# lvxianwei/DeepMerge

Hardware: NVIDIA B200
Metric: megapixels/sec end-to-end (RAG+pool+score+merge+relabel) (higher is better)
Workload: dtype int32/u8 index + fp32 scores

## Files before the change

### deepmerge_b200/csrc/rag_blocks.cu

```cuda
#include "rag_tables.cuh"

namespace dm {
namespace rag {
namespace blk {

template <int C_, int TH_, int NS_, int NW_, int ICAP_>
struct Cfg {
    static constexpr int C = C_, TH = TH_, NS = NS_, NWARPS = NW_, ICAP = ICAP_;
    static constexpr int CW = C_ > 0 ? C_ : 1;
    static constexpr int THREADS = NWARPS * 32;
    static constexpr int LAB_BOX = align128(TH * LAB_PITCH * 4);
    static constexpr int IMG_ROW_WORDS = STRIP_W * C / 4;
    static constexpr int IMG_BOX = align128(TH * IMG_ROW_WORDS * 4);
    static constexpr int STAGE_BYTES = LAB_BOX + IMG_BOX;
    static constexpr int ITEM_VECS = 7 + C;
    static constexpr int ITEM_BYTES = ICAP * ITEM_VECS * 16;
    static constexpr int TABLE_WORDS = RS * (3 + 2 * C) + ES * 3 + 4;
    static constexpr int TABLE_BYTES = align128(TABLE_WORDS * 4 + NS * 8);
    static constexpr int WARP_BYTES = NS * STAGE_BYTES + ITEM_BYTES + TABLE_BYTES;
    static constexpr int SMEM_BYTES = 128 + NWARPS * WARP_BYTES;
    static constexpr int TX_BYTES = TH * LAB_PITCH * 4 + (C > 0 ? TH * IMG_ROW_WORDS * 4 : 0);
    static constexpr int FLUSH_UNITS = FLUSH_ROWS / TH > 0 ? FLUSH_ROWS / TH : 1;
    static_assert(TH % 4 == 0, "a stage holds whole block rows");
    static_assert(ICAP % 8 == 0 && ICAP >= 40, "item buffer: the rest of a pass (< 32 items) plus a block row of new ones");
    static_assert(SMEM_BYTES <= 227 * 1024, "shared memory budget");
};

__device__ __noinline__ void slow_wait(uint64_t* bar, unsigned parity, unsigned long long* counters) {
    mbar_wait(bar, parity, counters);
}

template <typename CF>
__device__ __noinline__ void item_pass(uint4* items, unsigned* tab, const Params* Pp, int icount, int lane) {
    constexpr int C = CF::C, CW = CF::CW, ICAP = CF::ICAP;
    const Params& P = *Pp;
    const Tab<C> T = Tab<C>::from(tab);
    __syncwarp();
    const int n = min(32, icount), base = icount - n;
    if (lane < n) {
        const int j = base + lane;
        const uint4* it = items + j;
        int lab[ragcore::WIN];
        unsigned img[4 * CW];
        uint4 v = it[0];
        lab[20] = (int)v.x; lab[21] = (int)v.y; lab[22] = (int)v.z; lab[23] = (int)v.w;
#pragma unroll
        for (int r = 0; r < 4; ++r) {
            v = it[(1 + r) * ICAP];
            lab[5 * r] = (int)v.x; lab[5 * r + 1] = (int)v.y; lab[5 * r + 2] = (int)v.z; lab[5 * r + 3] = (int)v.w;
        }
        v = it[5 * ICAP];
        lab[4] = (int)v.x; lab[9] = (int)v.y; lab[14] = (int)v.z; lab[19] = (int)v.w;
#pragma unroll
        for (int vi = 0; vi < C; ++vi) {
            v = it[(6 + vi) * ICAP];
            img[4 * vi] = v.x; img[4 * vi + 1] = v.y; img[4 * vi + 2] = v.z; img[4 * vi + 3] = v.w;
        }
        v = it[(6 + C) * ICAP];
        const ragcore::Geo g{P.W, P.rows_own, P.rows_avail, P.top_border, P.bottom_border};
        Sink<C> sink{T, P};
        const ItemPick<ICAP> pick{(const int*)items, j};
        ragcore::process_item<C>(lab, img, (int)v.x, (int)v.y, g, sink, pick);
    }
    __syncwarp();
}

template <typename CF, bool USE_TMA>
__global__ void __launch_bounds__(CF::THREADS, 1)
rag_blocks_kernel(const __grid_constant__ CUtensorMap mapL, const __grid_constant__ CUtensorMap mapI,
                  const __grid_constant__ Params P) {
    constexpr int C = CF::C, CW = CF::CW, TH = CF::TH, NS = CF::NS, ICAP = CF::ICAP;
    extern __shared__ __align__(128) unsigned char smem_raw[];
    unsigned char* smem = smem_raw + ((128u - (smem_u32(smem_raw) & 127u)) & 127u);
    const int warp = __shfl_sync(0xffffffffu, (int)(threadIdx.x >> 5), 0);
    const int lane = threadIdx.x & 31;
    unsigned char* wbase = smem + (size_t)warp * CF::WARP_BYTES;
    uint4* items = (uint4*)(wbase + NS * CF::STAGE_BYTES);
    unsigned* tab = (unsigned*)(wbase + NS * CF::STAGE_BYTES + CF::ITEM_BYTES);
    const Tab<C> T = Tab<C>::from(tab);
    uint64_t* full_bar = (uint64_t*)(tab + ((CF::TABLE_WORDS + 1) & ~1));

    const long long total_units = (long long)P.tiles_x * P.tiles_y;
    const long long gw = (long long)blockIdx.x * CF::NWARPS + warp;
    const long long n_warps = (long long)gridDim.x * CF::NWARPS;
    const long long u_begin = total_units / n_warps * gw + min(gw, total_units % n_warps);
    const long long u_end = u_begin + total_units / n_warps + (gw < total_units % n_warps ? 1 : 0);
    const int my_units = (int)(u_end - u_begin);

    T.rkey[lane] = EMPTY_LABEL;
    T.rarea[lane] = 0;
    T.rborder[lane] = 0;
#pragma unroll
    for (int c = 0; c < C; ++c) {
        T.rsum[c * RS + lane] = 0;
        T.rsq[c * RS + lane] = 0;
    }
    T.ekey[lane] = EMPTY_KEY;
    T.ekey[lane + 32] = EMPTY_KEY;
    T.ecnt[lane] = 0;
    T.ecnt[lane + 32] = 0;
    if (lane == 0) {
        T.used[0] = T.used[1] = 0;
        if (USE_TMA) {
            for (int s = 0; s < NS; ++s) mbar_init(&full_bar[s], 1);
            asm volatile("fence.mbarrier_init.release.cluster;" ::: "memory");
        }
    }
    __syncwarp();
    if (my_units == 0) return;

    int isx = (int)(u_begin / P.tiles_y), ij = (int)(u_begin - (long long)isx * P.tiles_y), issued = 0;
    auto issue = [&]() {
        if (lane == 0) {
            const int st = issued % NS;
            unsigned char* sb = wbase + (size_t)st * CF::STAGE_BYTES;
            mbar_expect_tx(&full_bar[st], (unsigned)CF::TX_BYTES);
            tma_load_2d(sb, &mapL, isx * STRIP_W, ij * TH, &full_bar[st]);
            if (C > 0) tma_load_2d(sb + CF::LAB_BOX, &mapI, isx * STRIP_W * C / 4, ij * TH, &full_bar[st]);
        }
        ++issued;
        if (ij + 1 < P.tiles_y) ++ij;
        else { ij = 0; ++isx; }
    };
    if (USE_TMA) {
        for (int k = 0; k < NS && k < my_units; ++k) issue();
    }

    int4 up = make_int4(0, 0, 0, 0);
    int cur = EMPTY_LABEL;
    unsigned area = 0, s[CW], q[CW];
#pragma unroll
    for (int c = 0; c < CW; ++c) s[c] = q[c] = 0;
    int icount = 0;
    auto lane_flush = [&]() {
        if (cur >= 0 && area) table_region_add<C>(T, P, cur, area, 0u, s, q);
        area = 0;
#pragma unroll
        for (int c = 0; c < CW; ++c) s[c] = q[c] = 0;
    };

    int units_since_flush = 0;
    int sx = (int)(u_begin / P.tiles_y), j = (int)(u_begin - (long long)sx * P.tiles_y);
    bool contiguous = false;

    for (int i = 0; i < my_units; ++i) {
        const int st = USE_TMA ? i % NS : 0;
        unsigned char* sb = wbase + (size_t)st * CF::STAGE_BYTES;
        const int strip_x0 = sx * STRIP_W, unit_y0 = j * TH;
        int* Lw = (int*)sb;
        if (USE_TMA) {
            if (!mbar_try_wait(&full_bar[st], (unsigned)(i / NS) & 1u)) slow_wait(&full_bar[st], (unsigned)(i / NS) & 1u, P.counters);
        } else {
            __syncwarp();
            for (int k = lane; k < TH * LAB_PITCH; k += 32) {
                const int r = k / LAB_PITCH, cidx = k - r * LAB_PITCH;
                const int gy = unit_y0 + r, gx = strip_x0 + cidx;
                Lw[k] = (gy < P.rows_avail && gx < P.W) ? P.labels[(int64_t)gy * P.ld + gx] : 0;
            }
            if constexpr (C > 0) {
                unsigned char* Ib = sb + CF::LAB_BOX;
                for (int k = lane; k < TH * CF::IMG_ROW_WORDS * 4; k += 32) {
                    const int r = k / (CF::IMG_ROW_WORDS * 4), bidx = k - r * (CF::IMG_ROW_WORDS * 4);
                    const int gy = unit_y0 + r;
                    const int64_t gb = (int64_t)strip_x0 * C + bidx;
                    Ib[k] = (gy < P.rows_own && gb < (int64_t)P.W * C) ? P.image[(int64_t)gy * P.image_pitch + gb] : 0;
                }
            }
            __syncwarp();
        }

        const int x0 = strip_x0 + 4 * lane;
        const bool in_img = x0 < P.W;
        const bool forced_x = (x0 == 0) || (x0 + 4 >= P.W);
        if (!contiguous) {
            up = make_int4(0, 0, 0, 0);
            if (unit_y0 > 0) {
                const int32_t* row = P.labels + (int64_t)(unit_y0 - 1) * P.ld;
                if (x0 < P.W) up.x = row[x0];
                if (x0 + 1 < P.W) up.y = row[x0 + 1];
                if (x0 + 2 < P.W) up.z = row[x0 + 2];
                if (x0 + 3 < P.W) up.w = row[x0 + 3];
            }
        }

#pragma unroll
        for (int b = 0; b < TH / 4; ++b) {
            const int y0 = unit_y0 + 4 * b;
            if (y0 >= P.rows_avail) break;
            const int* Lp = Lw + (4 * b) * LAB_PITCH + 4 * lane;
            const int4 a0 = *(const int4*)Lp;
            const int4 a1 = *(const int4*)(Lp + LAB_PITCH);
            const int4 a2 = *(const int4*)(Lp + 2 * LAB_PITCH);
            const int4 a3 = *(const int4*)(Lp + 3 * LAB_PITCH);
            int r0 = __shfl_down_sync(0xffffffffu, a0.x, 1);
            int r1 = __shfl_down_sync(0xffffffffu, a1.x, 1);
            int r2 = __shfl_down_sync(0xffffffffu, a2.x, 1);
            int r3 = __shfl_down_sync(0xffffffffu, a3.x, 1);
            if (lane == 31) {
                r0 = Lp[4];
                r1 = Lp[LAB_PITCH + 4];
                r2 = Lp[2 * LAB_PITCH + 4];
                r3 = Lp[3 * LAB_PITCH + 4];
            }
            unsigned px[4][CW];
            if constexpr (C > 0) {
                const unsigned* Ip = (const unsigned*)(sb + CF::LAB_BOX) + (4 * b) * CF::IMG_ROW_WORDS + CW * lane;
#pragma unroll
                for (int r = 0; r < 4; ++r) {
                    if constexpr (C == 4) {
                        const uint4 v = *(const uint4*)(Ip + r * CF::IMG_ROW_WORDS);
                        px[r][0] = v.x; px[r][1] = v.y; px[r][2] = v.z; px[r][3] = v.w;
                    } else {
#pragma unroll
                        for (int c = 0; c < C; ++c) px[r][c] = Ip[r * CF::IMG_ROW_WORDS + c];
                    }
                }
            }
            const unsigned d = or3(or3(or3(eq3(up.x, up.y, up.z), eq3(up.z, up.w, a0.x), eq3(a0.x, a0.y, a0.z)),
                                       or3(eq3(a0.z, a0.w, r0), eq3(r0, a1.x, a1.y), eq3(a1.y, a1.z, a1.w)),
                                       or3(eq3(a1.w, r1, a2.x), eq3(a2.x, a2.y, a2.z), eq3(a2.z, a2.w, r2))),
                                   or3(eq3(r2, a3.x, a3.y), eq3(a3.y, a3.z, a3.w), eq3(a3.w, r3, up.x)), 0u);
            const bool forced = forced_x || (y0 == 0) || (y0 + 4 >= P.rows_own);
            const bool is_item = in_img && (forced || d != 0u);
            const bool is_fast = in_img && !is_item;
            const int ref = a0.x;
            if (is_fast && ref != cur) {
                lane_flush();
                cur = ref;
            }
            __syncwarp();
            if (is_fast) {
                area += 16u;
                if constexpr (C > 0) {
#pragma unroll
                    for (int r = 0; r < 4; ++r) ragcore::row_stats<C>(px[r], s, q);
                }
            }
            const unsigned bal = __ballot_sync(0xffffffffu, is_item);
            if (bal) {
                if (icount + __popc(bal) > ICAP) {
                    item_pass<CF>(items, tab, &P, icount, lane);
                    icount -= min(32, icount);
                }
                if (is_item) {
                    uint4* it = items + (icount + __popc(bal & lanemask_lt()));
                    it[0] = make_uint4((unsigned)up.x, (unsigned)up.y, (unsigned)up.z, (unsigned)up.w);
                    it[1 * ICAP] = make_uint4((unsigned)a0.x, (unsigned)a0.y, (unsigned)a0.z, (unsigned)a0.w);
                    it[2 * ICAP] = make_uint4((unsigned)a1.x, (unsigned)a1.y, (unsigned)a1.z, (unsigned)a1.w);
                    it[3 * ICAP] = make_uint4((unsigned)a2.x, (unsigned)a2.y, (unsigned)a2.z, (unsigned)a2.w);
                    it[4 * ICAP] = make_uint4((unsigned)a3.x, (unsigned)a3.y, (unsigned)a3.z, (unsigned)a3.w);
                    it[5 * ICAP] = make_uint4((unsigned)r0, (unsigned)r1, (unsigned)r2, (unsigned)r3);
                    if constexpr (C > 0) {
                        const unsigned* Wf = &px[0][0];
#pragma unroll
                        for (int vi = 0; vi < C; ++vi)
                            it[(6 + vi) * ICAP] = make_uint4(Wf[4 * vi], Wf[4 * vi + 1], Wf[4 * vi + 2], Wf[4 * vi + 3]);
                    }
                    it[(6 + C) * ICAP] = make_uint4((unsigned)x0, (unsigned)y0, 0u, 0u);
                }
                icount += __popc(bal);
            }
            up = a3;
        }
        contiguous = (j + 1 < P.tiles_y);

        if (j + 1 < P.tiles_y) ++j;
        else { j = 0; ++sx; }

        __syncwarp();
        if (USE_TMA && i + NS < my_units) {
            asm volatile("fence.proxy.async.shared::cta;" ::: "memory");
            issue();
        }

        ++units_since_flush;
        const bool forced_flush = units_since_flush >= CF::FLUSH_UNITS || (i + 1 == my_units);
        if (icount >= 32 || forced_flush) {
            while (icount >= 32 || (forced_flush && icount > 0)) {
                item_pass<CF>(items, tab, &P, icount, lane);
                icount -= min(32, icount);
                if (icount > 0 && (T.used[0] > RS / 2 || T.used[1] > ES / 2)) drain_tables<C>(tab, &P, lane);
            }
            if (forced_flush) {
                lane_flush();
                units_since_flush = 0;
            }
        }
        __syncwarp();
        const uint2 used = *(const uint2*)T.used;
        if (forced_flush || used.x > RS / 2 || used.y > ES / 2) drain_tables<C>(tab, &P, lane);
    }
}

template <typename CF>
static int run(const Params& Pin, cudaStream_t s) {
    Params P = Pin;
    P.tiles_x = (int)ceil_div(P.W, STRIP_W);
    P.tiles_y = (int)ceil_div(P.rows_avail, CF::TH);
    const long long total = (long long)P.tiles_x * P.tiles_y;
    if (total == 0) return DM_OK;
    const long long max_warps = (long long)num_sms() * CF::NWARPS;
    const long long per = ceil_div(total, max_warps);
    if (per > 0x7fffffff) return DM_ERR_BAD_ARG;
    P.tiles_per_cta = (int)per;
    const int grid = (int)imin64(num_sms(), ceil_div(total, CF::NWARPS));

    CUtensorMap mapL, mapI;
    memset(&mapL, 0, sizeof(mapL));
    memset(&mapI, 0, sizeof(mapI));
    bool tma = ((uintptr_t)P.labels % 16 == 0) && ((P.ld * 4) % 16 == 0) && P.ld >= P.W;
    if (CF::C > 0)
        tma = tma && ((uintptr_t)P.image % 16 == 0) && (P.image_pitch % 16 == 0) && (((int64_t)P.W * CF::C) % 4 == 0);
    if (tma)
        tma = make_map_2d(&mapL, P.labels, (uint64_t)P.W, (uint64_t)P.rows_avail, (uint64_t)P.ld * 4, LAB_PITCH, CF::TH);
    if (tma && CF::C > 0)
        tma = make_map_2d(&mapI, P.image, (uint64_t)P.W * CF::C / 4, (uint64_t)P.rows_own, (uint64_t)P.image_pitch,
                          CF::IMG_ROW_WORDS, CF::TH);
    set_last_path(tma ? 1 : 0);
    return launch(tma ? rag_blocks_kernel<CF, true> : rag_blocks_kernel<CF, false>, grid, CF::THREADS, CF::SMEM_BYTES, s,
                  mapL, mapI, P);
}

}

int run_blocks(const Params& P, int C, cudaStream_t s) {
    using namespace blk;
    switch (C) {
        case 0: return run<Cfg<0, 8, 2, 14, 48>>(P, s);
        case 1: return run<Cfg<1, 4, 2, 16, 48>>(P, s);
        case 2: return run<Cfg<2, 4, 2, 14, 48>>(P, s);
        case 3: return run<Cfg<3, 4, 2, 12, 48>>(P, s);
        case 4: return run<Cfg<4, 4, 2, 12, 48>>(P, s);
        default: return DM_ERR_BAD_ARG;
    }
}

}
}
```

### deepmerge_b200/csrc/rag_core.cuh

```cuda
#pragma once
#include <stdint.h>

#if defined(__CUDACC__)
#define DM_HD __host__ __device__ __forceinline__
#else
#define DM_HD inline
#endif

namespace dm {
namespace ragcore {

DM_HD unsigned popc32(unsigned x) {
#if defined(__CUDA_ARCH__)
    return (unsigned)__popc(x);
#else
    return (unsigned)__builtin_popcount(x);
#endif
}
DM_HD int ffs32(unsigned x) {
#if defined(__CUDA_ARCH__)
    return __ffs((int)x);
#else
    return x ? __builtin_ctz(x) + 1 : 0;
#endif
}
DM_HD unsigned dp4a_u8(unsigned a, unsigned b, unsigned c) {
#if defined(__CUDA_ARCH__)
    return __dp4a(a, b, c);
#else
    for (int i = 0; i < 4; ++i) c += ((a >> (8 * i)) & 0xffu) * ((b >> (8 * i)) & 0xffu);
    return c;
#endif
}
DM_HD unsigned byte_perm(unsigned a, unsigned b, unsigned s) {
#if defined(__CUDA_ARCH__)
    return __byte_perm(a, b, s);
#else
    const unsigned long long v = ((unsigned long long)b << 32) | a;
    unsigned r = 0;
    for (int i = 0; i < 4; ++i) r |= (unsigned)((v >> (8 * ((s >> (4 * i)) & 7))) & 0xffu) << (8 * i);
    return r;
#endif
}

constexpr int WIN = 24;
constexpr unsigned OWN_BITS = 0x7BDEFu;
constexpr unsigned COL0_BITS = 0x08421u;
constexpr unsigned RIGHT_BITS = 0x84210u;
DM_HD unsigned row_bits(int n) { return (1u << (5 * n)) - 1u; }

struct Geo {
    int W, rows_own, rows_avail, top_border, bottom_border;
};

struct BlockMasks {
    unsigned PV;
    unsigned SV;
    unsigned HV;
    unsigned VV;
    unsigned SIDES[4];
};

DM_HD int clamp04(int v) { return v < 0 ? 0 : (v > 4 ? 4 : v); }

DM_HD BlockMasks block_masks(int x0, int y0, const Geo& g) {
    BlockMasks m;
    const int ncols = clamp04(g.W - x0);
    const int nh = clamp04(g.W - x0 - 1);
    const int nown = clamp04(g.rows_own - y0);
    const int nav = clamp04(g.rows_avail - y0);
    const unsigned cols = ((1u << ncols) - 1u) * COL0_BITS;
    m.SV = cols & row_bits(nown);
    const unsigned ownv = cols & row_bits(nav);
    const unsigned rightv = (x0 + 4 < g.W) ? (RIGHT_BITS & row_bits(nown)) : 0u;
    const unsigned upv = (y0 > 0) ? (((1u << ncols) - 1u) << 20) : 0u;
    m.PV = ownv | rightv | upv;
    m.HV = (((1u << nh) - 1u) * COL0_BITS) & row_bits(nown);
    m.VV = ownv & ~(y0 > 0 ? 0u : 0x1Fu);
    const int klast = g.W - 1 - x0, rlast = g.rows_own - 1 - y0;
    m.SIDES[0] = x0 == 0 ? COL0_BITS : 0u;
    m.SIDES[1] = (klast >= 0 && klast < 4) ? (COL0_BITS << klast) : 0u;
    m.SIDES[2] = (y0 == 0 && g.top_border) ? 0xFu : 0u;
    m.SIDES[3] = (rlast >= 0 && rlast < 4 && g.rows_avail == g.rows_own && g.bottom_border) ? (0xFu << (5 * rlast)) : 0u;
    return m;
}

DM_HD bool block_forced(int x0, int y0, const Geo& g) {
    return x0 == 0 || x0 + 4 >= g.W || y0 == 0 || y0 + 4 >= g.rows_own;
}

DM_HD unsigned upper_of(unsigned M) { return (((M & OWN_BITS) << 5) & OWN_BITS) | ((M >> 20) & 0xFu); }

DM_HD unsigned pairs_between(unsigned A, unsigned B, const BlockMasks& m) {
    const unsigned h = ((A & (B >> 1)) | (B & (A >> 1))) & m.HV;
    const unsigned v = ((A & upper_of(B)) | (B & upper_of(A))) & m.VV;
    return popc32(h) + popc32(v);
}

DM_HD unsigned nibble_to_bytes(unsigned nib) { return ((nib * 0x00204081u) & 0x01010101u) * 0xFFu; }

template <int C>
DM_HD void band_transpose(const unsigned* W, unsigned* T) {
    if constexpr (C == 4) {
        const unsigned t0 = byte_perm(W[0], W[1], 0x5140), t1 = byte_perm(W[0], W[1], 0x7362);
        const unsigned t2 = byte_perm(W[2], W[3], 0x5140), t3 = byte_perm(W[2], W[3], 0x7362);
        T[0] = byte_perm(t0, t2, 0x5410);
        T[1] = byte_perm(t0, t2, 0x7632);
        T[2] = byte_perm(t1, t3, 0x5410);
        T[3] = byte_perm(t1, t3, 0x7632);
    } else {
#if defined(__CUDA_ARCH__)
#pragma unroll
#endif
        for (int c = 0; c < C; ++c) {
            const int i0 = c, i1 = C + c, i2 = 2 * C + c, i3 = 3 * C + c;
            const unsigned t01 = byte_perm(W[i0 >> 2], W[i1 >> 2], (unsigned)((i0 & 3) | ((4 + (i1 & 3)) << 4)));
            const unsigned t23 = byte_perm(W[i2 >> 2], W[i3 >> 2], (unsigned)((i2 & 3) | ((4 + (i3 & 3)) << 4)));
            T[c] = byte_perm(t01, t23, 0x5410);
        }
    }
}

template <int C>
DM_HD void row_stats(const unsigned* W, unsigned* s, unsigned* q) {
    unsigned T[C > 0 ? C : 1];
    band_transpose<C>(W, T);
#if defined(__CUDA_ARCH__)
#pragma unroll
#endif
    for (int c = 0; c < C; ++c) {
        s[c] = dp4a_u8(T[c], 0x01010101u, s[c]);
        q[c] = dp4a_u8(T[c], T[c], q[c]);
    }
}

DM_HD unsigned window_spread(const int* lab) {
    unsigned d = 0;
#if defined(__CUDA_ARCH__)
#pragma unroll
#endif
    for (int p = 1; p < WIN; p += 2) {
        const unsigned a = (unsigned)lab[p - 1], b = (unsigned)lab[p], c = (unsigned)lab[(p + 1) % WIN];
        d |= (a ^ b) | (b ^ c);
    }
    return d;
}

template <int C, class Sink, class Pick>
DM_HD void process_item(const int* lab, const unsigned* img , int x0, int y0, const Geo& g, Sink& sink,
                        const Pick& pick) {
    constexpr int CW = C > 0 ? C : 1;
    const BlockMasks m = block_masks(x0, y0, g);

    unsigned MN = 0;
    {
        int any = 0;
#if defined(__CUDA_ARCH__)
#pragma unroll
#endif
        for (int p = 0; p < WIN; ++p) any |= lab[p];
        if (any < 0) {
#if defined(__CUDA_ARCH__)
#pragma unroll
#endif
            for (int p = 0; p < WIN; ++p) MN |= (lab[p] < 0 ? 1u : 0u) << p;
            MN &= m.PV;
        }
    }

    unsigned T[4][CW];
    if (C > 0) {
#if defined(__CUDA_ARCH__)
#pragma unroll
#endif
        for (int r = 0; r < 4; ++r) band_transpose<C>(img + r * CW, T[r]);
    }

    constexpr int MAXL = 4;
    unsigned rem = m.PV & ~MN;
    int Lq1 = 0, Lq2 = 0, Lq3 = 0;
    unsigned Mq1 = 0, Mq2 = 0, Mq3 = 0;
#if defined(__CUDA_ARCH__)
#pragma unroll 1
#endif
    for (int i = 0; i < MAXL && rem != 0; ++i) {
        const int l = pick(ffs32(rem) - 1);
        unsigned mm = 0;
#if defined(__CUDA_ARCH__)
#pragma unroll
#endif
        for (int p = 0; p < WIN; ++p) mm |= (lab[p] == l ? 1u : 0u) << p;
        mm &= rem;
        rem &= ~mm;
        {
            const unsigned ms = mm & m.SV;
            unsigned sides = popc32(ms & m.SIDES[0]) + popc32(ms & m.SIDES[1]) + popc32(ms & m.SIDES[2]) +
                             popc32(ms & m.SIDES[3]);
            if (MN) sides += pairs_between(mm, MN, m);
            unsigned s[CW], q[CW];
#if defined(__CUDA_ARCH__)
#pragma unroll
#endif
            for (int c = 0; c < CW; ++c) s[c] = q[c] = 0;
            if (C > 0) {
#if defined(__CUDA_ARCH__)
#pragma unroll
#endif
                for (int r = 0; r < 4; ++r) {
                    const unsigned bm = nibble_to_bytes((ms >> (5 * r)) & 0xFu);
#if defined(__CUDA_ARCH__)
#pragma unroll
#endif
                    for (int c = 0; c < C; ++c) {
                        const unsigned w = T[r][c] & bm;
                        s[c] = dp4a_u8(w, 0x01010101u, s[c]);
                        q[c] = dp4a_u8(w, w, q[c]);
                    }
                }
            }
            const unsigned area = popc32(ms);
            if (area | sides) sink.region(l, area, sides, s, q);
        }
#if defined(__CUDA_ARCH__)
#pragma unroll 1
#endif
        for (int j = 0; j < 3; ++j) {
            if (Mq1) {
                const unsigned n = pairs_between(mm, Mq1, m);
                if (n) sink.edge(l, Lq1, n);
            }
            const int tl = Lq1;
            const unsigned tm = Mq1;
            Lq1 = Lq2; Mq1 = Mq2;
            Lq2 = Lq3; Mq2 = Mq3;
            Lq3 = tl; Mq3 = tm;
        }
        Lq3 = Lq2; Mq3 = Mq2;
        Lq2 = Lq1; Mq2 = Mq1;
        Lq1 = l; Mq1 = mm;
    }
    if (rem == 0) return;

#if defined(__CUDA_ARCH__)
#pragma unroll
#endif
    for (int r = 0; r < 4; ++r) {
#if defined(__CUDA_ARCH__)
#pragma unroll 1
#endif
        for (int k = 0; k < 4; ++k) {
            const int p = 5 * r + k;
            const unsigned bit = 1u << p;
            const int l = pick(p);
            if ((m.SV & rem & bit) && l >= 0) {
                unsigned s[CW], q[CW];
                for (int c = 0; c < CW; ++c) s[c] = q[c] = 0;
                if (C > 0) {
                    const unsigned bm = 0xFFu << (8 * k);
                    for (int c = 0; c < C; ++c) {
                        const unsigned w = T[r][c] & bm;
                        s[c] = dp4a_u8(w, 0x01010101u, 0u);
                        q[c] = dp4a_u8(w, w, 0u);
                    }
                }
                const unsigned sides = ((m.SIDES[0] & bit) ? 1u : 0u) + ((m.SIDES[1] & bit) ? 1u : 0u) +
                                       ((m.SIDES[2] & bit) ? 1u : 0u) + ((m.SIDES[3] & bit) ? 1u : 0u);
                sink.region_slow(l, 1u, sides, s, q);
            }
            for (int which = 0; which < 2; ++which) {
                const bool ok = which == 0 ? (m.HV & bit) != 0 : (m.VV & bit) != 0;
                if (!ok) continue;
                const int po = which == 0 ? p + 1 : (r == 0 ? 20 + k : p - 5);
                if (((bit | (1u << po)) & rem) == 0) continue;
                const int o = pick(po);
                if (o == l) continue;
                if ((o | l) >= 0) {
                    sink.edge_slow(l, o, 1u);
                } else {
                    const int v = l >= 0 ? l : o;
                    if (v >= 0) {
                        unsigned z[CW];
                        for (int c = 0; c < CW; ++c) z[c] = 0;
                        sink.region_slow(v, 0u, 1u, z, z);
                    }
                }
            }
        }
    }
}

}
}
```

### deepmerge_b200/csrc/rag_tables.cuh

```cuda
#pragma once
#include "rag_common.cuh"
#include "rag_core.cuh"

namespace dm {
namespace rag {
namespace blk {

template <int C>
struct Tab {
    int* rkey;
    unsigned* rarea;
    unsigned* rborder;
    unsigned* rsum;
    unsigned* rsq;
    unsigned long long* ekey;
    unsigned* ecnt;
    unsigned* used;
    unsigned* base;

    __device__ __forceinline__ static Tab from(unsigned* tab) {
        Tab T;
        T.base = tab;
        T.rkey = (int*)tab;
        T.rarea = tab + RS;
        T.rborder = tab + 2 * RS;
        T.rsum = tab + 3 * RS;
        T.rsq = tab + (3 + C) * RS;
        T.ekey = (unsigned long long*)(tab + (3 + 2 * C) * RS);
        T.ecnt = tab + (3 + 2 * C) * RS + 2 * ES;
        T.used = tab + (3 + 2 * C) * RS + 3 * ES;
        return T;
    }
};

__device__ __forceinline__ unsigned eq3(int a, int b, int c) {
    unsigned d;
    asm("lop3.b32 %0, %1, %2, %3, 0x7E;" : "=r"(d) : "r"(a), "r"(b), "r"(c));
    return d;
}
__device__ __forceinline__ unsigned or3(unsigned a, unsigned b, unsigned c) {
    unsigned d;
    asm("lop3.b32 %0, %1, %2, %3, 0xFE;" : "=r"(d) : "r"(a), "r"(b), "r"(c));
    return d;
}
__device__ __forceinline__ void red_add_u64(unsigned long long* p, unsigned long long v) {
    asm volatile("red.global.add.u64 [%0], %1;" ::"l"(p), "l"(v) : "memory");
}

__device__ __forceinline__ int region_slot(int* rkey, unsigned* used, int label) {
    unsigned h = ((unsigned)label * 0x9E3779B1u) >> (32 - 5);
    static_assert(RS == 32, "hash shift");
#pragma unroll 1
    for (int p = 0; p < RS; ++p) {
        int k = rkey[h];
        if (k == label) return (int)h;
        if (k == EMPTY_LABEL) {
            int old = atomicCAS(&rkey[h], EMPTY_LABEL, label);
            if (old == EMPTY_LABEL) {
                atomicAdd(&used[0], 1u);
                return (int)h;
            }
            if (old == label) return (int)h;
        }
        h = (h + 1) & (RS - 1);
    }
    return SLOT_NONE;
}

__device__ __forceinline__ void raw_append(const Params& P, unsigned long long key, unsigned cnt) {
    if ((long long)key_hi(key) >= P.n_regions) {
        atomicExch(&P.counters[3], 1ull);
        return;
    }
    unsigned long long i = atomicAdd(&P.counters[1], 1ull);
    if ((long long)i < P.capacity) {
        P.raw_keys[i] = key;
        P.raw_cnt[i] = cnt;
    } else {
        atomicExch(&P.counters[2], 1ull);
    }
}

template <int C>
__device__ __forceinline__ void edge_add(const Tab<C>& T, const Params& P, unsigned long long key, unsigned cnt) {
    unsigned h = (((unsigned)(key >> 32) * 0x9E3779B1u) ^ ((unsigned)key * 0x85EBCA6Bu)) >> (32 - 6);
    static_assert(ES == 64, "hash shift");
#pragma unroll 1
    for (int p = 0; p < ES / 2; ++p) {
        unsigned long long k = T.ekey[h];
        if (k == EMPTY_KEY) {
            k = atomicCAS(&T.ekey[h], EMPTY_KEY, key);
            if (k == EMPTY_KEY) {
                atomicAdd(&T.used[1], 1u);
                k = key;
            }
        }
        if (k == key) {
            atomicAdd(&T.ecnt[h], cnt);
            return;
        }
        h = (h + 1) & (ES - 1);
    }
    raw_append(P, key, cnt);
}

template <int C>
__device__ __forceinline__ void global_region_add(const Params& P, int label, unsigned area, unsigned border,
                                                  const unsigned* s, const unsigned* q) {
    if ((unsigned)label >= (unsigned)P.n_regions) {
        atomicExch(&P.counters[3], 1ull);
        return;
    }
    if (area) red_add_u64(&P.area[label], (unsigned long long)area);
    if (border) red_add_u64(&P.border[label], (unsigned long long)border);
    if (C > 0 && area) {
#pragma unroll
        for (int c = 0; c < C; ++c) {
            red_add_u64(&P.bsum[(size_t)label * C + c], (unsigned long long)s[c]);
            red_add_u64(&P.bsq[(size_t)label * C + c], (unsigned long long)q[c]);
        }
    }
}

template <int C>
__device__ __noinline__ void global_region_add_slow(const Params* P, int label, unsigned area, unsigned border, uint4 s4,
                                                    uint4 q4) {
    const unsigned s[4] = {s4.x, s4.y, s4.z, s4.w}, q[4] = {q4.x, q4.y, q4.z, q4.w};
    global_region_add<C>(*P, label, area, border, s, q);
}

template <int C>
__device__ __forceinline__ void table_region_add(const Tab<C>& T, const Params& P, int label, unsigned area,
                                                 unsigned border, const unsigned* s, const unsigned* q) {
    const int slot = region_slot(T.rkey, T.used, label);
    if (slot >= 0) {
        if (area) atomicAdd(&T.rarea[slot], area);
        if (border) atomicAdd(&T.rborder[slot], border);
        if (C > 0 && area) {
#pragma unroll
            for (int c = 0; c < C; ++c) {
                atomicAdd(&T.rsum[c * RS + slot], s[c]);
                atomicAdd(&T.rsq[c * RS + slot], q[c]);
            }
        }
    } else {
        uint4 s4 = make_uint4(0, 0, 0, 0), q4 = make_uint4(0, 0, 0, 0);
        if (C > 0) { s4.x = s[0]; q4.x = q[0]; }
        if (C > 1) { s4.y = s[1 % (C > 0 ? C : 1)]; q4.y = q[1 % (C > 0 ? C : 1)]; }
        if (C > 2) { s4.z = s[2 % (C > 0 ? C : 1)]; q4.z = q[2 % (C > 0 ? C : 1)]; }
        if (C > 3) { s4.w = s[3 % (C > 0 ? C : 1)]; q4.w = q[3 % (C > 0 ? C : 1)]; }
        global_region_add_slow<C>(&P, label, area, border, s4, q4);
    }
}

template <int C>
__device__ __noinline__ void slow_edge_add(unsigned* tab, const Params* P, int a, int b, unsigned cnt) {
    edge_add<C>(Tab<C>::from(tab), *P, pack_key(a, b), cnt);
}
template <int C>
__device__ __noinline__ void slow_region_add(unsigned* tab, const Params* P, int label, unsigned area, unsigned border,
                                             uint4 s4, uint4 q4) {
    const unsigned s[4] = {s4.x, s4.y, s4.z, s4.w}, q[4] = {q4.x, q4.y, q4.z, q4.w};
    table_region_add<C>(Tab<C>::from(tab), *P, label, area, border, s, q);
}

template <int C>
struct Sink {
    const Tab<C>& T;
    const Params& P;
    __device__ __forceinline__ void region(int l, unsigned area, unsigned sides, const unsigned* s, const unsigned* q) const {
        table_region_add<C>(T, P, l, area, sides, s, q);
    }
    __device__ __forceinline__ void edge(int a, int b, unsigned n) const { edge_add<C>(T, P, pack_key(a, b), n); }
    __device__ __forceinline__ void region_slow(int l, unsigned area, unsigned sides, const unsigned* s,
                                                const unsigned* q) const {
        uint4 s4 = make_uint4(0, 0, 0, 0), q4 = make_uint4(0, 0, 0, 0);
        if (C > 0) { s4.x = s[0]; q4.x = q[0]; }
        if (C > 1) { s4.y = s[1 % (C > 0 ? C : 1)]; q4.y = q[1 % (C > 0 ? C : 1)]; }
        if (C > 2) { s4.z = s[2 % (C > 0 ? C : 1)]; q4.z = q[2 % (C > 0 ? C : 1)]; }
        if (C > 3) { s4.w = s[3 % (C > 0 ? C : 1)]; q4.w = q[3 % (C > 0 ? C : 1)]; }
        slow_region_add<C>(T.base, &P, l, area, sides, s4, q4);
    }
    __device__ __forceinline__ void edge_slow(int a, int b, unsigned n) const { slow_edge_add<C>(T.base, &P, a, b, n); }
};

template <int ICAP>
struct ItemPick {
    const int* words;
    int j;
    __device__ __forceinline__ int operator()(int p) const {
        const int r = (p * 13) >> 6;
        const int k = p - 5 * r;
        const int vec = p >= 20 ? 0 : (k == 4 ? 5 : 1 + r);
        const int w = p >= 20 ? p - 20 : (k == 4 ? r : k);
        return words[(vec * ICAP + j) * 4 + w];
    }
};

template <int C>
__device__ __forceinline__ void drain_tables_impl(unsigned* tab, const Params* Pp, int lane) {
    constexpr int CW = C > 0 ? C : 1;
    const Tab<C> T = Tab<C>::from(tab);
    const Params& P = *Pp;
    static_assert(RS == 32 && ES == 64, "one / two slots per lane");
    __syncwarp();
    {
        const int label = T.rkey[lane];
        if (label != EMPTY_LABEL) {
            unsigned s[CW], q[CW];
#pragma unroll
            for (int c = 0; c < C; ++c) {
                s[c] = T.rsum[c * RS + lane];
                q[c] = T.rsq[c * RS + lane];
                T.rsum[c * RS + lane] = 0;
                T.rsq[c * RS + lane] = 0;
            }
            global_region_add<C>(P, label, T.rarea[lane], T.rborder[lane], s, q);
            T.rkey[lane] = EMPTY_LABEL;
            T.rarea[lane] = 0;
            T.rborder[lane] = 0;
        }
    }
#pragma unroll
    for (int k0 = 0; k0 < ES; k0 += 32) {
        const int k = k0 + lane;
        unsigned long long key = T.ekey[k];
        unsigned cnt = 0;
        if (key != EMPTY_KEY) {
            cnt = T.ecnt[k];
            T.ekey[k] = EMPTY_KEY;
            T.ecnt[k] = 0;
            if ((long long)key_hi(key) >= P.n_regions) {
                atomicExch(&P.counters[3], 1ull);
                key = EMPTY_KEY;
            }
        }
        const bool has = key != EMPTY_KEY;
        const unsigned bal = __ballot_sync(0xffffffffu, has);
        if (bal) {
            unsigned long long base = 0;
            if (lane == 0) base = atomicAdd(&P.counters[1], (unsigned long long)__popc(bal));
            base = __shfl_sync(0xffffffffu, base, 0);
            if (has) {
                const unsigned long long idx = base + __popc(bal & lanemask_lt());
                if ((long long)idx < P.capacity) {
                    P.raw_keys[idx] = key;
                    P.raw_cnt[idx] = cnt;
                } else {
                    atomicExch(&P.counters[2], 1ull);
                }
            }
        }
    }
    if (lane == 0) T.used[0] = T.used[1] = 0;
    __syncwarp();
}

template <int C>
__device__ __noinline__ void drain_tables(unsigned* tab, const Params* Pp, int lane) {
    drain_tables_impl<C>(tab, Pp, lane);
}

template <int C>
struct InlineSink {
    const Tab<C>& T;
    const Params& P;
    __device__ __forceinline__ void region(int l, unsigned area, unsigned sides, const unsigned* s, const unsigned* q) const {
        const int slot = region_slot(T.rkey, T.used, l);
        if (slot >= 0) {
            if (area) atomicAdd(&T.rarea[slot], area);
            if (sides) atomicAdd(&T.rborder[slot], sides);
            if (C > 0 && area) {
#pragma unroll
                for (int c = 0; c < C; ++c) {
                    atomicAdd(&T.rsum[c * RS + slot], s[c]);
                    atomicAdd(&T.rsq[c * RS + slot], q[c]);
                }
            }
        } else {
            global_region_add<C>(P, l, area, sides, s, q);
        }
    }
    __device__ __forceinline__ void edge(int a, int b, unsigned n) const { edge_add<C>(T, P, pack_key(a, b), n); }
    __device__ __forceinline__ void region_slow(int l, unsigned area, unsigned sides, const unsigned* s,
                                                const unsigned* q) const {
        region(l, area, sides, s, q);
    }
    __device__ __forceinline__ void edge_slow(int a, int b, unsigned n) const { edge(a, b, n); }
};

}
}
}
```

Before: 122,300.

## Prefetch image bytes into registers instead of TMA staging; read item windows from smem

Drops the TMA image tile and its shared-memory stage, and instead has each lane load its 4x4 block's image bytes straight from global memory into registers one unit ahead, using non-allocating streaming loads. item_pass no longer copies the label window and image into local arrays. process_item now reads them lazily from the shared item buffer through accessor objects, and band transposes are done per row on demand. The smaller shared footprint lets the image configs run 16 warps with a smaller item buffer. The cost is extra register pressure and global-load latency, plus reloading labels and image after a mid-row item flush.

```diff
diff --git a/deepmerge_b200/csrc/rag_blocks.cu b/deepmerge_b200/csrc/rag_blocks.cu
--- a/deepmerge_b200/csrc/rag_blocks.cu
+++ b/deepmerge_b200/csrc/rag_blocks.cu
@@ -9,66 +9,95 @@
     static constexpr int C = C_, TH = TH_, NS = NS_, NWARPS = NW_, ICAP = ICAP_;
     static constexpr int CW = C_ > 0 ? C_ : 1;
     static constexpr int THREADS = NWARPS * 32;
-    static constexpr int LAB_BOX = align128(TH * LAB_PITCH * 4);
-    static constexpr int IMG_ROW_WORDS = STRIP_W * C / 4;
-    static constexpr int IMG_BOX = align128(TH * IMG_ROW_WORDS * 4);
-    static constexpr int STAGE_BYTES = LAB_BOX + IMG_BOX;
+    static constexpr int STAGE_BYTES = align128(TH * LAB_PITCH * 4);
     static constexpr int ITEM_VECS = 7 + C;
     static constexpr int ITEM_BYTES = ICAP * ITEM_VECS * 16;
     static constexpr int TABLE_WORDS = RS * (3 + 2 * C) + ES * 3 + 4;
     static constexpr int TABLE_BYTES = align128(TABLE_WORDS * 4 + NS * 8);
     static constexpr int WARP_BYTES = NS * STAGE_BYTES + ITEM_BYTES + TABLE_BYTES;
     static constexpr int SMEM_BYTES = 128 + NWARPS * WARP_BYTES;
-    static constexpr int TX_BYTES = TH * LAB_PITCH * 4 + (C > 0 ? TH * IMG_ROW_WORDS * 4 : 0);
+    static constexpr int TX_BYTES = TH * LAB_PITCH * 4;
     static constexpr int FLUSH_UNITS = FLUSH_ROWS / TH > 0 ? FLUSH_ROWS / TH : 1;
     static_assert(TH % 4 == 0, "a stage holds whole block rows");
+    static_assert(C == 0 || TH == 4, "image bytes are prefetched one unit = one block row ahead");
     static_assert(ICAP % 8 == 0 && ICAP >= 40, "item buffer: the rest of a pass (< 32 items) plus a block row of new ones");
     static_assert(SMEM_BYTES <= 227 * 1024, "shared memory budget");
 };
 
+__device__ __forceinline__ uint4 ldg_stream_v4(const void* p) {
+    uint4 v;
+    asm volatile("ld.global.nc.L1::no_allocate.v4.u32 {%0, %1, %2, %3}, [%4];"
+                 : "=r"(v.x), "=r"(v.y), "=r"(v.z), "=r"(v.w) : "l"(p));
+    return v;
+}
+__device__ __forceinline__ uint2 ldg_stream_v2(const void* p) {
+    uint2 v;
+    asm volatile("ld.global.nc.L1::no_allocate.v2.u32 {%0, %1}, [%2];" : "=r"(v.x), "=r"(v.y) : "l"(p));
+    return v;
+}
+__device__ __forceinline__ unsigned ldg_stream(const void* p) {
+    unsigned v;
+    asm volatile("ld.global.nc.L1::no_allocate.u32 %0, [%1];" : "=r"(v) : "l"(p));
+    return v;
+}
+
+template <int C, bool ALIGNED>
+__device__ __forceinline__ void load_block_image(unsigned (&px)[4][C], const Params& P, int x0, int y0) {
+    const int nb = min(4 * C, (P.W - x0) * C);
+#pragma unroll
+    for (int r = 0; r < 4; ++r) {
+        const uint8_t* row = P.image + (int64_t)(y0 + r) * P.image_pitch + (int64_t)x0 * C;
+#pragma unroll
+        for (int w = 0; w < C; ++w) px[r][w] = 0;
+        if (y0 + r >= P.rows_own || nb <= 0) continue;
+        if (ALIGNED && nb == 4 * C) {
+            if constexpr (C == 4) {
+                const uint4 v = ldg_stream_v4(row);
+                px[r][0] = v.x; px[r][1] = v.y; px[r][2] = v.z; px[r][3] = v.w;
+            } else if constexpr (C == 2) {
+                const uint2 v = ldg_stream_v2(row);
+                px[r][0] = v.x; px[r][1] = v.y;
+            } else {
+#pragma unroll
+                for (int w = 0; w < C; ++w) px[r][w] = ldg_stream(row + 4 * w);
+            }
+        } else if (ALIGNED) {
+#pragma unroll
+            for (int w = 0; w < C; ++w)
+                if (4 * w < nb) px[r][w] = ldg_stream(row + 4 * w);
+        } else {
+#pragma unroll
+            for (int b = 0; b < 4 * C; ++b)
+                if (b < nb) px[r][b >> 2] |= (unsigned)row[b] << (8 * (b & 3));
+        }
+    }
+}
+
 __device__ __noinline__ void slow_wait(uint64_t* bar, unsigned parity, unsigned long long* counters) {
     mbar_wait(bar, parity, counters);
 }
 
 template <typename CF>
 __device__ __noinline__ void item_pass(uint4* items, unsigned* tab, const Params* Pp, int icount, int lane) {
-    constexpr int C = CF::C, CW = CF::CW, ICAP = CF::ICAP;
+    constexpr int C = CF::C, ICAP = CF::ICAP;
     const Params& P = *Pp;
     const Tab<C> T = Tab<C>::from(tab);
     __syncwarp();
     const int n = min(32, icount), base = icount - n;
     if (lane < n) {
         const int j = base + lane;
-        const uint4* it = items + j;
-        int lab[ragcore::WIN];
-        unsigned img[4 * CW];
-        uint4 v = it[0];
-        lab[20] = (int)v.x; lab[21] = (int)v.y; lab[22] = (int)v.z; lab[23] = (int)v.w;
-#pragma unroll
-        for (int r = 0; r < 4; ++r) {
-            v = it[(1 + r) * ICAP];
-            lab[5 * r] = (int)v.x; lab[5 * r + 1] = (int)v.y; lab[5 * r + 2] = (int)v.z; lab[5 * r + 3] = (int)v.w;
-        }
-        v = it[5 * ICAP];
-        lab[4] = (int)v.x; lab[9] = (int)v.y; lab[14] = (int)v.z; lab[19] = (int)v.w;
-#pragma unroll
-        for (int vi = 0; vi < C; ++vi) {
-            v = it[(6 + vi) * ICAP];
-            img[4 * vi] = v.x; img[4 * vi + 1] = v.y; img[4 * vi + 2] = v.z; img[4 * vi + 3] = v.w;
-        }
-        v = it[(6 + C) * ICAP];
+        const uint4 v = items[(6 + C) * ICAP + j];
         const ragcore::Geo g{P.W, P.rows_own, P.rows_avail, P.top_border, P.bottom_border};
         Sink<C> sink{T, P};
-        const ItemPick<ICAP> pick{(const int*)items, j};
-        ragcore::process_item<C>(lab, img, (int)v.x, (int)v.y, g, sink, pick);
+        const ItemPick<ICAP> win{(const int*)items, j};
+        ragcore::process_item<C>(win, win, (int)v.x, (int)v.y, g, sink, win);
     }
     __syncwarp();
 }
 
 template <typename CF, bool USE_TMA>
 __global__ void __launch_bounds__(CF::THREADS, 1)
-rag_blocks_kernel(const __grid_constant__ CUtensorMap mapL, const __grid_constant__ CUtensorMap mapI,
-                  const __grid_constant__ Params P) {
+rag_blocks_kernel(const __grid_constant__ CUtensorMap mapL, const __grid_constant__ Params P) {
     constexpr int C = CF::C, CW = CF::CW, TH = CF::TH, NS = CF::NS, ICAP = CF::ICAP;
     extern __shared__ __align__(128) unsigned char smem_raw[];
     unsigned char* smem = smem_raw + ((128u - (smem_u32(smem_raw) & 127u)) & 127u);
@@ -109,21 +138,18 @@
     __syncwarp();
     if (my_units == 0) return;
 
-    int isx = (int)(u_begin / P.tiles_y), ij = (int)(u_begin - (long long)isx * P.tiles_y), issued = 0;
-    auto issue = [&]() {
+    int isx = (int)(u_begin / P.tiles_y), ij = (int)(u_begin - (long long)isx * P.tiles_y);
+    auto issue = [&](int st) {
         if (lane == 0) {
-            const int st = issued % NS;
             unsigned char* sb = wbase + (size_t)st * CF::STAGE_BYTES;
             mbar_expect_tx(&full_bar[st], (unsigned)CF::TX_BYTES);
             tma_load_2d(sb, &mapL, isx * STRIP_W, ij * TH, &full_bar[st]);
-            if (C > 0) tma_load_2d(sb + CF::LAB_BOX, &mapI, isx * STRIP_W * C / 4, ij * TH, &full_bar[st]);
-        }
-        ++issued;
+        }
         if (ij + 1 < P.tiles_y) ++ij;
         else { ij = 0; ++isx; }
     };
     if (USE_TMA) {
-        for (int k = 0; k < NS && k < my_units; ++k) issue();
+        for (int k = 0; k < NS && k < my_units; ++k) issue(k);
     }
 
     int4 up = make_int4(0, 0, 0, 0);
@@ -139,15 +165,27 @@
         for (int c = 0; c < CW; ++c) s[c] = q[c] = 0;
     };
 
-    int units_since_flush = 0;
     int sx = (int)(u_begin / P.tiles_y), j = (int)(u_begin - (long long)sx * P.tiles_y);
     bool contiguous = false;
+    unsigned pxn[4][CW];
+    if constexpr (C > 0) load_block_image<C, USE_TMA>(pxn, P, sx * STRIP_W + 4 * lane, j * TH);
 
     for (int i = 0; i < my_units; ++i) {
         const int st = USE_TMA ? i % NS : 0;
         unsigned char* sb = wbase + (size_t)st * CF::STAGE_BYTES;
         const int strip_x0 = sx * STRIP_W, unit_y0 = j * TH;
         int* Lw = (int*)sb;
+        unsigned px[4][CW];
+        if constexpr (C > 0) {
+#pragma unroll
+            for (int r = 0; r < 4; ++r)
+#pragma unroll
+                for (int c = 0; c < C; ++c) px[r][c] = pxn[r][c];
+            if (i + 1 < my_units) {
+                const bool last = j + 1 == P.tiles_y;
+                load_block_image<C, USE_TMA>(pxn, P, (last ? sx + 1 : sx) * STRIP_W + 4 * lane, last ? 0 : (j + 1) * TH);
+            }
+        }
         if (USE_TMA) {
             if (!mbar_try_wait(&full_bar[st], (unsigned)(i / NS) & 1u)) slow_wait(&full_bar[st], (unsigned)(i / NS) & 1u, P.counters);
         } else {
@@ -156,15 +194,6 @@
                 const int r = k / LAB_PITCH, cidx = k - r * LAB_PITCH;
                 const int gy = unit_y0 + r, gx = strip_x0 + cidx;
                 Lw[k] = (gy < P.rows_avail && gx < P.W) ? P.labels[(int64_t)gy * P.ld + gx] : 0;
-            }
-            if constexpr (C > 0) {
-                unsigned char* Ib = sb + CF::LAB_BOX;
-                for (int k = lane; k < TH * CF::IMG_ROW_WORDS * 4; k += 32) {
-                    const int r = k / (CF::IMG_ROW_WORDS * 4), bidx = k - r * (CF::IMG_ROW_WORDS * 4);
-                    const int gy = unit_y0 + r;
-                    const int64_t gb = (int64_t)strip_x0 * C + bidx;
-                    Ib[k] = (gy < P.rows_own && gb < (int64_t)P.W * C) ? P.image[(int64_t)gy * P.image_pitch + gb] : 0;
-                }
             }
             __syncwarp();
         }
@@ -188,10 +217,10 @@
             const int y0 = unit_y0 + 4 * b;
             if (y0 >= P.rows_avail) break;
             const int* Lp = Lw + (4 * b) * LAB_PITCH + 4 * lane;
-            const int4 a0 = *(const int4*)Lp;
-            const int4 a1 = *(const int4*)(Lp + LAB_PITCH);
-            const int4 a2 = *(const int4*)(Lp + 2 * LAB_PITCH);
-            const int4 a3 = *(const int4*)(Lp + 3 * LAB_PITCH);
+            int4 a0 = *(const int4*)Lp;
+            int4 a1 = *(const int4*)(Lp + LAB_PITCH);
+            int4 a2 = *(const int4*)(Lp + 2 * LAB_PITCH);
+            int4 a3 = *(const int4*)(Lp + 3 * LAB_PITCH);
             int r0 = __shfl_down_sync(0xffffffffu, a0.x, 1);
             int r1 = __shfl_down_sync(0xffffffffu, a1.x, 1);
             int r2 = __shfl_down_sync(0xffffffffu, a2.x, 1);
@@ -201,20 +230,6 @@
                 r1 = Lp[LAB_PITCH + 4];
                 r2 = Lp[2 * LAB_PITCH + 4];
                 r3 = Lp[3 * LAB_PITCH + 4];
-            }
-            unsigned px[4][CW];
-            if constexpr (C > 0) {
-                const unsigned* Ip = (const unsigned*)(sb + CF::LAB_BOX) + (4 * b) * CF::IMG_ROW_WORDS + CW * lane;
-#pragma unroll
-                for (int r = 0; r < 4; ++r) {
-                    if constexpr (C == 4) {
-                        const uint4 v = *(const uint4*)(Ip + r * CF::IMG_ROW_WORDS);
-                        px[r][0] = v.x; px[r][1] = v.y; px[r][2] = v.z; px[r][3] = v.w;
-                    } else {
-#pragma unroll
-                        for (int c = 0; c < C; ++c) px[r][c] = Ip[r * CF::IMG_ROW_WORDS + c];
-                    }
-                }
             }
             const unsigned d = or3(or3(or3(eq3(up.x, up.y, up.z), eq3(up.z, up.w, a0.x), eq3(a0.x, a0.y, a0.z)),
                                        or3(eq3(a0.z, a0.w, r0), eq3(r0, a1.x, a1.y), eq3(a1.y, a1.z, a1.w)),
@@ -241,6 +256,16 @@
                 if (icount + __popc(bal) > ICAP) {
                     item_pass<CF>(items, tab, &P, icount, lane);
                     icount -= min(32, icount);
+                    a0 = *(const int4*)Lp;
+                    a1 = *(const int4*)(Lp + LAB_PITCH);
+                    a2 = *(const int4*)(Lp + 2 * LAB_PITCH);
+                    a3 = *(const int4*)(Lp + 3 * LAB_PITCH);
+                    r0 = Lp[4];
+                    r1 = Lp[LAB_PITCH + 4];
+                    r2 = Lp[2 * LAB_PITCH + 4];
+                    r3 = Lp[3 * LAB_PITCH + 4];
+                    if constexpr (C > 0)
+                        if (is_item) load_block_image<C, USE_TMA>(px, P, x0, y0);
                 }
                 if (is_item) {
                     uint4* it = items + (icount + __popc(bal & lanemask_lt()));
@@ -270,21 +295,17 @@
         __syncwarp();
         if (USE_TMA && i + NS < my_units) {
             asm volatile("fence.proxy.async.shared::cta;" ::: "memory");
-            issue();
-        }
-
-        ++units_since_flush;
-        const bool forced_flush = units_since_flush >= CF::FLUSH_UNITS || (i + 1 == my_units);
+            issue(st);
+        }
+
+        const bool forced_flush = (i + 1) % CF::FLUSH_UNITS == 0 || (i + 1 == my_units);
         if (icount >= 32 || forced_flush) {
             while (icount >= 32 || (forced_flush && icount > 0)) {
                 item_pass<CF>(items, tab, &P, icount, lane);
                 icount -= min(32, icount);
                 if (icount > 0 && (T.used[0] > RS / 2 || T.used[1] > ES / 2)) drain_tables<C>(tab, &P, lane);
             }
-            if (forced_flush) {
-                lane_flush();
-                units_since_flush = 0;
-            }
+            if (forced_flush) lane_flush();
         }
         __syncwarp();
         const uint2 used = *(const uint2*)T.used;
@@ -305,20 +326,16 @@
     P.tiles_per_cta = (int)per;
     const int grid = (int)imin64(num_sms(), ceil_div(total, CF::NWARPS));
 
-    CUtensorMap mapL, mapI;
+    CUtensorMap mapL;
     memset(&mapL, 0, sizeof(mapL));
-    memset(&mapI, 0, sizeof(mapI));
     bool tma = ((uintptr_t)P.labels % 16 == 0) && ((P.ld * 4) % 16 == 0) && P.ld >= P.W;
     if (CF::C > 0)
         tma = tma && ((uintptr_t)P.image % 16 == 0) && (P.image_pitch % 16 == 0) && (((int64_t)P.W * CF::C) % 4 == 0);
     if (tma)
         tma = make_map_2d(&mapL, P.labels, (uint64_t)P.W, (uint64_t)P.rows_avail, (uint64_t)P.ld * 4, LAB_PITCH, CF::TH);
-    if (tma && CF::C > 0)
-        tma = make_map_2d(&mapI, P.image, (uint64_t)P.W * CF::C / 4, (uint64_t)P.rows_own, (uint64_t)P.image_pitch,
-                          CF::IMG_ROW_WORDS, CF::TH);
     set_last_path(tma ? 1 : 0);
     return launch(tma ? rag_blocks_kernel<CF, true> : rag_blocks_kernel<CF, false>, grid, CF::THREADS, CF::SMEM_BYTES, s,
-                  mapL, mapI, P);
+                  mapL, P);
 }
 
 }
@@ -327,10 +344,10 @@
     using namespace blk;
     switch (C) {
         case 0: return run<Cfg<0, 8, 2, 14, 48>>(P, s);
-        case 1: return run<Cfg<1, 4, 2, 16, 48>>(P, s);
-        case 2: return run<Cfg<2, 4, 2, 14, 48>>(P, s);
-        case 3: return run<Cfg<3, 4, 2, 12, 48>>(P, s);
-        case 4: return run<Cfg<4, 4, 2, 12, 48>>(P, s);
+        case 1: return run<Cfg<1, 4, 2, 16, 40>>(P, s);
+        case 2: return run<Cfg<2, 4, 2, 16, 40>>(P, s);
+        case 3: return run<Cfg<3, 4, 2, 16, 40>>(P, s);
+        case 4: return run<Cfg<4, 4, 2, 16, 40>>(P, s);
         default: return DM_ERR_BAD_ARG;
     }
 }
diff --git a/deepmerge_b200/csrc/rag_core.cuh b/deepmerge_b200/csrc/rag_core.cuh
--- a/deepmerge_b200/csrc/rag_core.cuh
+++ b/deepmerge_b200/csrc/rag_core.cuh
@@ -146,35 +146,41 @@
     return d;
 }
 
-template <int C, class Sink, class Pick>
-DM_HD void process_item(const int* lab, const unsigned* img , int x0, int y0, const Geo& g, Sink& sink,
-                        const Pick& pick) {
+DM_HD unsigned label_mask(const int* lab, int l) {
+    unsigned mm = 0;
+#if defined(__CUDA_ARCH__)
+#pragma unroll
+#endif
+    for (int p = 0; p < WIN; ++p) mm |= (lab[p] == l ? 1u : 0u) << p;
+    return mm;
+}
+DM_HD unsigned nodata_mask(const int* lab) {
+    int any = 0;
+#if defined(__CUDA_ARCH__)
+#pragma unroll
+#endif
+    for (int p = 0; p < WIN; ++p) any |= lab[p];
+    unsigned mn = 0;
+    if (any < 0) {
+#if defined(__CUDA_ARCH__)
+#pragma unroll
+#endif
+        for (int p = 0; p < WIN; ++p) mn |= (lab[p] < 0 ? 1u : 0u) << p;
+    }
+    return mn;
+}
+template <int C>
+DM_HD void image_row(const unsigned* img, int r, unsigned* w) {
+    constexpr int CW = C > 0 ? C : 1;
+    for (int c = 0; c < CW; ++c) w[c] = img[r * CW + c];
+}
+
+template <int C, class Win, class Img, class Sink, class Pick>
+DM_HD void process_item(Win lab, Img img, int x0, int y0, const Geo& g, Sink& sink, const Pick& pick) {
     constexpr int CW = C > 0 ? C : 1;
     const BlockMasks m = block_masks(x0, y0, g);
 
-    unsigned MN = 0;
-    {
-        int any = 0;
-#if defined(__CUDA_ARCH__)
-#pragma unroll
-#endif
-        for (int p = 0; p < WIN; ++p) any |= lab[p];
-        if (any < 0) {
-#if defined(__CUDA_ARCH__)
-#pragma unroll
-#endif
-            for (int p = 0; p < WIN; ++p) MN |= (lab[p] < 0 ? 1u : 0u) << p;
-            MN &= m.PV;
-        }
-    }
-
-    unsigned T[4][CW];
-    if (C > 0) {
-#if defined(__CUDA_ARCH__)
-#pragma unroll
-#endif
-        for (int r = 0; r < 4; ++r) band_transpose<C>(img + r * CW, T[r]);
-    }
+    const unsigned MN = nodata_mask(lab) & m.PV;
 
     constexpr int MAXL = 4;
     unsigned rem = m.PV & ~MN;
@@ -185,12 +191,7 @@
 #endif
     for (int i = 0; i < MAXL && rem != 0; ++i) {
         const int l = pick(ffs32(rem) - 1);
-        unsigned mm = 0;
-#if defined(__CUDA_ARCH__)
-#pragma unroll
-#endif
-        for (int p = 0; p < WIN; ++p) mm |= (lab[p] == l ? 1u : 0u) << p;
-        mm &= rem;
+        const unsigned mm = label_mask(lab, l) & rem;
         rem &= ~mm;
         {
             const unsigned ms = mm & m.SV;
@@ -207,12 +208,15 @@
 #pragma unroll
 #endif
                 for (int r = 0; r < 4; ++r) {
+                    unsigned W[CW], T[CW];
+                    image_row<C>(img, r, W);
+                    band_transpose<C>(W, T);
                     const unsigned bm = nibble_to_bytes((ms >> (5 * r)) & 0xFu);
 #if defined(__CUDA_ARCH__)
 #pragma unroll
 #endif
                     for (int c = 0; c < C; ++c) {
-                        const unsigned w = T[r][c] & bm;
+                        const unsigned w = T[c] & bm;
                         s[c] = dp4a_u8(w, 0x01010101u, s[c]);
                         q[c] = dp4a_u8(w, w, q[c]);
                     }
@@ -256,9 +260,12 @@
                 unsigned s[CW], q[CW];
                 for (int c = 0; c < CW; ++c) s[c] = q[c] = 0;
                 if (C > 0) {
+                    unsigned W[CW], T[CW];
+                    image_row<C>(img, r, W);
+                    band_transpose<C>(W, T);
                     const unsigned bm = 0xFFu << (8 * k);
                     for (int c = 0; c < C; ++c) {
-                        const unsigned w = T[r][c] & bm;
+                        const unsigned w = T[c] & bm;
                         s[c] = dp4a_u8(w, 0x01010101u, 0u);
                         q[c] = dp4a_u8(w, w, 0u);
                     }
diff --git a/deepmerge_b200/csrc/rag_tables.cuh b/deepmerge_b200/csrc/rag_tables.cuh
--- a/deepmerge_b200/csrc/rag_tables.cuh
+++ b/deepmerge_b200/csrc/rag_tables.cuh
@@ -195,7 +195,49 @@
         const int w = p >= 20 ? p - 20 : (k == 4 ? r : k);
         return words[(vec * ICAP + j) * 4 + w];
     }
+    template <class F>
+    __device__ __forceinline__ unsigned mask(F f) const {
+        const uint4* it = (const uint4*)words + j;
+        uint4 v = it[0];
+        unsigned m = (f((int)v.x) << 20) | (f((int)v.y) << 21) | (f((int)v.z) << 22) | (f((int)v.w) << 23);
+#pragma unroll
+        for (int r = 0; r < 4; ++r) {
+            v = it[(1 + r) * ICAP];
+            m |= (f((int)v.x) | (f((int)v.y) << 1) | (f((int)v.z) << 2) | (f((int)v.w) << 3)) << (5 * r);
+        }
+        v = it[5 * ICAP];
+        return m | (f((int)v.x) << 4) | (f((int)v.y) << 9) | (f((int)v.z) << 14) | (f((int)v.w) << 19);
+    }
 };
+
+template <int ICAP>
+__device__ __forceinline__ unsigned label_mask(const ItemPick<ICAP>& w, int l) {
+    return w.mask([l](int v) { return v == l ? 1u : 0u; });
+}
+template <int ICAP>
+__device__ __forceinline__ unsigned nodata_mask(const ItemPick<ICAP>& w) {
+    const uint4* it = (const uint4*)w.words + w.j;
+    unsigned any = 0;
+#pragma unroll
+    for (int v = 0; v < 6; ++v) {
+        const uint4 x = it[v * ICAP];
+        any |= x.x | x.y | x.z | x.w;
+    }
+    return (int)any < 0 ? w.mask([](int v) { return (unsigned)v >> 31; }) : 0u;
+}
+template <int C, int ICAP>
+__device__ __forceinline__ void image_row(const ItemPick<ICAP>& it, int r, unsigned* w) {
+    if constexpr (C == 4) {
+        const uint4 v = ((const uint4*)it.words)[(6 + r) * ICAP + it.j];
+        w[0] = v.x; w[1] = v.y; w[2] = v.z; w[3] = v.w;
+    } else {
+#pragma unroll
+        for (int c = 0; c < C; ++c) {
+            const int k = r * C + c;
+            w[c] = (unsigned)it.words[((6 + k / 4) * ICAP + it.j) * 4 + k % 4];
+        }
+    }
+}
 
 template <int C>
 __device__ __forceinline__ void drain_tables_impl(unsigned* tab, const Params* Pp, int lane) {
```

Result: slower. 117,600, median of 6 (-3.9%).
